# nncarlson/nka

Hardware: AMD Instinct MI355X
Metric: NKA updates/sec + achieved HBM GB/s at n=1e8, m=20 fp64; 1/2/4/8 GPUs (higher is better)
Workload: dtype f64

## Files before the change

### include/nka_hip_diag.h

```cpp
#ifndef NKA_HIP_DIAG_H
#define NKA_HIP_DIAG_H

#include "nka_hip_ext.h"
#include "nka_hip_vec.h"

#ifdef __cplusplus
extern "C" {
#endif

int nka_hip_set_tuning(nka_hip_t a, const char *key, int32_t value);

int nka_hip_set_grid(nka_hip_t a, int32_t pa_blocks_per_cu, int32_t pb_blocks_per_cu);

int nka_hip_debug_time_pa(nka_hip_t a, const double *f_dev, int32_t reps, float *ms_mean);

int nka_hip_debug_chain_sum(nka_hip_t a, const double *x_dev, const double *y_dev, int64_t n, double start, int32_t walk,
                            double *sum, float *ms);

int nka_hip_get_stamps(nka_hip_t a, double *out16);

int nka_hip_vec_set_tuning(nka_hip_vec_ws_t ws, const char *key, int32_t value);

#ifdef __cplusplus
}
#endif
// ... 2 lines not shown
```

### nka_amd/_lib.py

```python
from __future__ import annotations

import ctypes as C
import os
import subprocess

HERE = os.path.dirname(os.path.abspath(__file__))
_LIB = None

_i32p = C.POINTER(C.c_int32)
_dp = C.POINTER(C.c_double)
ALLREDUCE_FN = C.CFUNCTYPE(C.c_int, C.c_void_p, C.c_void_p, C.c_int32, C.c_void_p)
HOST_DOT_FN = C.CFUNCTYPE(C.c_double, C.c_void_p, C.c_int64, C.POINTER(C.c_double), C.POINTER(C.c_double))
HOST_ALLREDUCE_FN = C.CFUNCTYPE(C.c_int, C.c_void_p, C.POINTER(C.c_double), C.c_int32)

SIGNATURES = {
    "nka_hip_create": (C.c_int, [C.POINTER(C.c_void_p), C.c_int64, C.c_int32, C.c_double, C.c_int32, C.c_int32, C.c_void_p]),
    "nka_hip_destroy": (C.c_int, [C.c_void_p]),
    "nka_hip_clone": (C.c_int, [C.c_void_p, C.POINTER(C.c_void_p)]),
    "nka_hip_capture_safe": (C.c_int, [C.c_void_p]),
    "nka_hip_list_bound": (C.c_int, [C.c_void_p]),
    "nka_hip_set_stream": (C.c_int, [C.c_void_p, C.c_void_p]),
    "nka_hip_accel_update": (C.c_int, [C.c_void_p, C.c_void_p]),
    "nka_hip_accel_update_host": (C.c_int, [C.c_void_p, C.c_void_p]),
    "nka_hip_accel_update_swap": (C.c_int, [C.c_void_p, C.POINTER(C.c_void_p), C.POINTER(C.c_void_p)]),
# ... 109 lines not shown
    "nka_hip_batch_get_state": (C.c_int, [C.c_void_p, C.c_int32, _i32p, _i32p, _i32p, _i32p, _i32p, _i32p, _i32p, _dp, _dp]),
    "nka_hip_batch_get_reductions": (C.c_int, [C.c_void_p, C.c_int32, _dp]),
    "nka_hip_batch_get_w": (C.c_int, [C.c_void_p, C.c_int32, C.c_int32, _dp]),
    "nka_hip_batch_get_v": (C.c_int, [C.c_void_p, C.c_int32, C.c_int32, _dp]),
    "nka_hip_batch_state_digest": (C.c_int, [C.c_void_p, C.c_int32, C.POINTER(C.c_uint64)]),
}


DIAG_SIGNATURES = {
    "nka_hip_set_tuning": (C.c_int, [C.c_void_p, C.c_char_p, C.c_int32]),
    "nka_hip_set_grid": (C.c_int, [C.c_void_p, C.c_int32, C.c_int32]),
    "nka_hip_debug_time_pa": (C.c_int, [C.c_void_p, C.c_void_p, C.c_int32, C.POINTER(C.c_float)]),
    "nka_hip_debug_chain_sum": (C.c_int, [C.c_void_p, C.c_void_p, C.c_void_p, C.c_int64, C.c_double, C.c_int32,
                                          C.POINTER(C.c_double), C.POINTER(C.c_float)]),
    "nka_hip_get_stamps": (C.c_int, [C.c_void_p, _dp]),
    "nka_hip_vec_set_tuning": (C.c_int, [C.c_void_p, C.c_char_p, C.c_int32]),
}
_DIAG = None


def diag_lib_path() -> str:
    return os.environ.get("NKA_HIP_DIAG_LIB") or os.path.join(HERE, "libnka_hip_diag.so")


def load_diag() -> C.CDLL:
    global _DIAG
    if _DIAG is None:
        path = diag_lib_path()
        if not os.path.exists(path):
            raise RuntimeError(f"{path} not found: `make -C nka_amd/csrc diag` (or __graft_entry__.build())")
# ... 54 lines not shown
```

### nka_amd/csrc/handles.hpp

```cpp
#pragma once

#include "../../include/nka_hip.h"
#include "../../include/nka_hip_ext.h"
#include "../../include/nka_hip_vec.h"
#include "nka_ctl.hpp"
#include "host_logic.hpp"
#include "rccl_dl.hpp"

#include <hip/hip_runtime.h>

#include <cstdint>
#include <string>
#include <vector>

namespace nka_detail {
int set_error(int code, const std::string &msg);
std::string last_error();
bool &span_check_failed();
int check_device_span(const void *p, int64_t n, const char *what);
int check_device_span_i32(const void *p, int64_t n, const char *what);
void invalidate_span_cache();
void register_allocation(const void *p, size_t bytes, const void *owner);
void unregister_owner(const void *owner);
void unregister_allocation(const void *p);
// ... 51 lines not shown
  int num_cu = 256;
  int bpc[2] = {0, 0};
  char devname[64] = {0};
  int pa_pipe = -1;
  int pb_pipe = -1;
  int pb_flags = 0;
  int pb_tile = -1;
  int pb_tickets = -1;
  double *chain_pred = nullptr;
  void *chain_summ = nullptr;
  long long chain_cap = 0;
  int chain_many = -1;
  int chain_walk = 0;
  int fail_after_solve = 0;
  int prime_pad = -1;
  bool state_in_global = false;
  bool serial_solve = false;
  int sum_order = NKA_HIP_SUMS_AUTO;
  bool debug = false;
  nka_hip_allreduce_fn allreduce = nullptr;
  void *allreduce_ctx = nullptr;
  ncclComm_t comm = nullptr;
  nka::P2P p2p{};
  void *p2p_mail = nullptr;
  std::vector<void *> p2p_opened;
  void *p2p_dev = nullptr;
  int p2p_ranks = 0;
  bool p2p_fused = false;
  int pa_normed = 0;
  int shard_rank = -1, shard_n = 0;
// ... 32 lines not shown
```

### nka_amd/csrc/lab.hip

```cpp
#include "handles.hpp"
#include "nka_chain.hpp"
#include "../../include/nka_hip_diag.h"

#include <algorithm>
#include <string>

using namespace nka;
using namespace nka_detail;

extern "C" {

int nka_hip_get_stamps(nka_hip_t a, double *out16) {
  if (!a || !out16) return fail(NKA_HIP_EINVAL, "null argument");
  HIP_TRY(hipSetDevice(a->device));
  HIP_TRY(hipMemcpyAsync(out16, a->ctl.stamps(), sizeof(double) * kStamps, hipMemcpyDeviceToHost, a->stream));
  HIP_TRY(hipStreamSynchronize(a->stream));
  return 0;
}

int nka_hip_set_grid(nka_hip_t a, int32_t pa, int32_t pb) {
  if (!a) return fail(NKA_HIP_EINVAL, "null handle");
  const int32_t v[2] = {pa, pb};
  for (int i = 0; i < 2; i++) {
    if (v[i] < 0 || v[i] * a->num_cu > kMaxGrid) return fail(NKA_HIP_EINVAL, "blocks per CU out of range");
    a->bpc[i] = v[i];
  }
  return 0;
}

int nka_hip_debug_chain_sum(nka_hip_t a, const double *x, const double *y, int64_t n, double start, int32_t walk, double *sum,
// ... 69 lines not shown
    if (value != -1 && value != 0 && !(value > 200 && value <= 204))
      return fail(NKA_HIP_EINVAL, "pa_pipe: -1 (auto), 0 (every load of a tile in flight), 201..204 (rolling window, 1..4 blocks per CU)");
    a->pa_pipe = value;
  } else if (k == "pb_tile") {
    if (value != -1 && value != 1 && value != 2) return fail(NKA_HIP_EINVAL, "pb_tile: -1 (auto), 1, 2");
    a->pb_tile = value;
  } else if (k == "pb_tickets") {
    if (value != -1 && value != 0 && value != 1 && value != 2 && value != 4 && value != 8)
      return fail(NKA_HIP_EINVAL, "pb_tickets: -1 (auto), 0 (static tile mapping), 1, 2, 4, 8 (ticket counters)");
    a->pb_tickets = value;
  } else if (k == "fail_after_solve") {
    a->fail_after_solve = value != 0;
  } else if (k == "prime_pad") {
    if (value < -1 || value > 1) return fail(NKA_HIP_EINVAL, "prime_pad: -1, 0, 1");
    a->prime_pad = value;
  } else if (k == "chain_many") {
    if (value < -1 || value > 1) return fail(NKA_HIP_EINVAL, "chain_many: -1, 0, 1");
    a->chain_many = value;
  } else if (k == "chain_walk") {
    a->chain_walk = value != 0;
  } else if (k == "serial_solve") {
    a->serial_solve = value != 0;
  } else if (k == "list_word") {
    a->word_off = value == 0;
  } else {
    return fail(NKA_HIP_EINVAL, "unknown tuning key: " + k);
  }
  return 0;
}

// ... 13 lines not shown
```

### nka_amd/csrc/nka_ctl.hpp

```cpp
#pragma once

#include <cstddef>
#include <cstdint>

#if defined(__HIPCC__)
#include <hip/hip_runtime.h>
#define NKA_HOST_DEVICE __host__ __device__
#else
#define NKA_HOST_DEVICE
#endif

namespace nka {

enum {
  IC_SUBSPACE = 0,
  IC_PENDING = 1,
  IC_FIRST = 2,
  IC_LAST = 3,
  IC_FREE = 4,
  IC_NEW = 5,
  IC_NCOMB = 6,
  IC_PLAN_PENDING = 7,
  IC_PLAN_FIRST = 8,
  IC_PLAN_NOLDER = 9,
  IC_NRELAX = 10,
  IC_NORMED = 11,
  IC_HEADER = 16
};
enum { DC_VTOL = 0, DC_S = 1, DC_HEADER = 2 };
enum {
  PC_FIRST_W = 0,
  PC_NEW_W = 1,
  PC_NEW_V = 2,
  PC_OLD_W = 3,
  PC_OLD_V = 4,
  PC_WGT = 5,
  PC_HEADER = 8
};

constexpr int kMaxPerPass = 32;

// ... 54 lines not shown
```

### nka_amd/csrc/nka_device.hpp

```cpp
#pragma once

#include "nka_ctl.hpp"

#include <hip/hip_runtime.h>
#include <stdint.h>

#if defined(__HIP_DEVICE_COMPILE__) && !defined(__gfx950__)
#error "nka_device.hpp is written for gfx950 (CDNA4) only: v_permlane32_swap / v_permlane16_swap reductions, 160 KiB LDS, tile shapes measured on MI355X.  Build with --offload-arch=gfx950."
#endif

namespace nka {

constexpr int kBlock = 256;
constexpr int kWavesPerBlock = kBlock / 64;
constexpr int kMaxGrid = 4096;

#ifdef NKA_SOLVE_STAMPS
#define NKA_STAMP(ctl, i) do { if (threadIdx.x == 0) (ctl).stamps()[i] = (double)__builtin_amdgcn_s_memtime(); } while (0)
#define NKA_STAMP0(ctl, i) do { if (blockIdx.x == 0 && threadIdx.x == 0) (ctl).stamps()[i] = (double)__builtin_amdgcn_s_memtime(); } while (0)
#else
#define NKA_STAMP(ctl, i) do { } while (0)
#define NKA_STAMP0(ctl, i) do { } while (0)
#endif

// ... 144 lines not shown
  return __builtin_nontemporal_load(reinterpret_cast<const d2 *>(p));
}
__device__ __forceinline__ void st(double *p, double x) { __builtin_nontemporal_store(x, p); }
__device__ __forceinline__ void st(double *p, d2 x) { __builtin_nontemporal_store(x, reinterpret_cast<d2 *>(p)); }

__device__ __forceinline__ double ex(double x, int) { return x; }
__device__ __forceinline__ double ex(d2 x, int i) { return x[i]; }
__device__ __forceinline__ void setc(double &x, int, double val) { x = val; }
__device__ __forceinline__ void setc(d2 &x, int i, double val) { x[i] = val; }

__device__ __forceinline__ double pa_operand(double d, int normed, double s, double rs) {
  if (normed == 0) return d;
  if (s == 0.0) return 0.0;
  return (normed & 2) ? rs * d : d / s;
}

template <bool WGT, class V>
__device__ __forceinline__ double wgt_first(const V &om, int q, double a) {
  if constexpr (WGT) return ex(om, q) * a;
  else return a;
}
template <bool WGT>
__device__ __forceinline__ double wgt_at(const double *__restrict__ wgt, int64_t i, double a) {
  if constexpr (WGT) return wgt[i] * a;
  else return a;
}

constexpr int kOrdThreads = 256;
constexpr int kOrdChunkMax = 512;
constexpr int kOrdMaxMvec = 250;
// ... 269 lines not shown
```

### nka_amd/csrc/nka_hip.hip

```cpp
#include "handles.hpp"
#include "nka_kernels.hpp"

#include <dlfcn.h>

#include <algorithm>
#include <atomic>
#include <chrono>
#include <cmath>
#include <cstdio>
#include <cstdlib>
#include <cstring>
#include <map>
#include <mutex>
#include <set>
#include <string>
#include <vector>

using namespace nka;

namespace {
thread_local std::string g_err;
}

namespace nka_detail {
// ... 176 lines not shown
  else
    hipLaunchKernelGGL((k_dots<MAXL, VEC>), dim3(g), dim3(kBlock), 0, a->stream, a->ctl, a->vs, f, a->partials, pass, a->pa_normed);
  hipLaunchKernelGGL((k_finalize_dots<MAXL>), dim3(2 * MAXL + 2), dim3(kFinThreads), 0, a->stream, a->ctl,
                     a->partials, g, pass, npass * MAXL, pass * MAXL, a->p2p_fused ? a->p2p : P2P{}, a->pa_normed ? 1 : 0);
  return g;
}

template <int MAXL, int W>
int launch_dots_win_1(const nka_hip_state *a, const double *f, int bpc, int base, int pass, int ncover) {
  static const int occ = occupancy_of(k_dots_win<MAXL, W>);
  const int64_t ntile = a->n / (kBlock * 2);
  int64_t g = (int64_t)a->num_cu * std::min(occ, std::max(1, bpc));
  g = std::max<int64_t>(1, std::min<int64_t>(std::min<int64_t>(g, std::max<int64_t>(ntile, 1)), kMaxGrid));
  if (a->weighted)
    hipLaunchKernelGGL((k_dots_win<MAXL, W, true>), dim3((int)g), dim3(kBlock), 0, a->stream, a->ctl, a->vs, f, a->partials, base,
                       a->pa_normed);
  else
    hipLaunchKernelGGL((k_dots_win<MAXL, W>), dim3((int)g), dim3(kBlock), 0, a->stream, a->ctl, a->vs, f, a->partials, base, a->pa_normed);
  hipLaunchKernelGGL((k_finalize_dots<MAXL>), dim3(2 * MAXL + 2), dim3(kFinThreads), 0, a->stream, a->ctl,
                     a->partials, (int)g, pass, ncover < 0 ? MAXL : ncover, base, a->p2p_fused ? a->p2p : P2P{}, a->pa_normed ? 1 : 0);
  return (int)g;
}

template <int MAXL>
constexpr int win_ring() {
  return MAXL % 4 == 0 ? 4 : MAXL % 5 == 0 ? 5 : MAXL % 6 == 0 ? 6 : MAXL % 3 == 0 ? 3 : MAXL % 7 == 0 ? 7 : MAXL;
}

template <int MAXK>
constexpr int win_ring_pairs() {
  return MAXK % 2 == 0 ? 2 : MAXK % 3 == 0 ? 3 : MAXK % 5 == 0 ? 5 : MAXK % 7 == 0 ? 7 : MAXK;
}

#ifndef NKA_WINDOW_WIDTH_STEP
#define NKA_WINDOW_WIDTH_STEP 1
// ... 414 lines not shown
    e = hipGetLastError();
  }
  if (e != hipSuccess) {
    nka_hip_destroy(b);
    return fail(NKA_HIP_EHIP, std::string("nka_hip_clone: ") + hipGetErrorString(e));
  }
  b->pending = src->pending;
  b->list_ub = src->list_ub;
  b->bpc[0] = src->bpc[0];
  b->bpc[1] = src->bpc[1];
  b->pa_pipe = src->pa_pipe;
  b->pb_pipe = src->pb_pipe;
  b->pb_tile = src->pb_tile;
  b->pb_tickets = src->pb_tickets;
  b->prime_pad = src->prime_pad;
  b->chain_walk = src->chain_walk;
  b->chain_many = src->chain_many;
  b->chain_pred = nullptr; b->chain_summ = nullptr; b->chain_cap = 0;
  b->serial_solve = src->serial_solve;
  b->sum_order = src->sum_order;
  b->shard_rank = src->shard_rank;
  b->shard_n = src->shard_n;
  b->debug = src->debug;
  if (src->allreduce != rccl_allreduce && src->allreduce != p2p_allreduce) {
    b->allreduce = src->allreduce;
    b->allreduce_ctx = src->allreduce_ctx;
    b->needs_comm = src->needs_comm;
  } else {
    b->needs_comm = true;
  }
// ... 44 lines not shown
    if (a->relaxed_after.size() > 4096) a->relaxed_after.erase(a->relaxed_after.begin(), a->relaxed_after.begin() + 2048);
  }
  return 0;
}

int nka_hip_set_vec_tol(nka_hip_t a, double vtol) {
  if (!a) return fail(NKA_HIP_EINVAL, "null handle");
  if (!(vtol > 0.0)) return fail(NKA_HIP_EINVAL, "set_vec_tol: vtol must be > 0");
  HIP_TRY(hipSetDevice(a->device));
  a->vtol = vtol;
  HIP_TRY(hipMemcpyAsync(a->ctl.dc + DC_VTOL, &a->vtol, sizeof(double), hipMemcpyHostToDevice, a->stream));
  HIP_TRY(hipStreamSynchronize(a->stream));
  return 0;
}

static int enqueue_solve(nka_hip_t a, int mode, long long swap_w = kNoBuffer, long long swap_v = kNoBuffer, bool gather = false) {
  hipStream_t s = a->stream;
  const P2P x = gather ? a->p2p : P2P{};
  if (a->mvec + 1 <= kSolveWaveMax && !a->serial_solve) {
    const size_t sm = solve_wave_smem_bytes(a->mvec);
    const int nl = a->mvec + 1;
    const long long id_stride = (a->swapped || a->captured) ? 0 : (long long)a->vs.stride, id_vbase = buffer_offset(a, a->vs.v);
#define ROWS(NL) \
  hipLaunchKernelGGL((k_solve_rows<NL>), dim3(1), dim3(kSolveThreads), sm, s, a->ctl, mode, swap_w, swap_v, id_stride, id_vbase, x)
    if (nl <= 6) ROWS(6);
    else if (nl <= 11) ROWS(11);
    else if (nl <= 21) ROWS(21);
    else if (nl <= 33) ROWS(33);
    else if (nl <= 48) ROWS(48);
    else {
      if (!a->solve63_raised) {
        const hipError_t raised = hipFuncSetAttribute(reinterpret_cast<const void *>(k_solve_rows<63>),
                                                      hipFuncAttributeMaxDynamicSharedMemorySize,
                                                      (int)solve_wave_smem_bytes(kSolveWaveMax - 1));
        if (raised != hipSuccess) return fail(NKA_HIP_EHIP, std::string("raising the dynamic LDS limit failed: ") + hipGetErrorString(raised));
        a->solve63_raised = true;
      }
      ROWS(63);
    }
// ... 393 lines not shown
  a->p2p_fused = r.gather;
  enqueue_pa(a, f, vec, older_ub);
  a->p2p_fused = false;
  if (hipError_t e = hipGetLastError(); e != hipSuccess) {
    r.rc = fail(NKA_HIP_EHIP, std::string("accel_update: ") + hipGetErrorString(e));
    return r;
  }
  if (a->allreduce && !r.gather)
    if (int rc = a->allreduce(a->allreduce_ctx, a->ctl.red(), a->ctl.red_count(), a->stream)) r.rc = hook_failed(rc);
  return r;
}

static int update_impl(nka_hip_t a, double *f, long long swap_w, long long swap_v);
static int p2p_status_after_sync(nka_hip_t a);

int nka_hip_accel_update(nka_hip_t a, double *f) { return update_impl(a, f, kNoBuffer, kNoBuffer); }

static int update_impl(nka_hip_t a, double *f, long long swap_w, long long swap_v) {
  if (!a) return fail(NKA_HIP_EINVAL, "null handle");
  if (!f && a->n > 0) return fail(NKA_HIP_EINVAL, "accel_update: f is NULL");
  HIP_TRY(hipSetDevice(a->device));
  if (int rc = nka_detail::check_device_span(f, a->n, "accel_update: f")) return rc;
  if (swap_w == kNoBuffer && f && f == a->last_acc)
    return fail(NKA_HIP_EINVAL, "accel_update: that buffer is the accelerated f lent by the previous out-of-place update (read only: "
                                "it is the stored v of the pending pair); copy it, or go on with nka_hip_accel_update_swap");
  if (a->poisoned)
    return fail(NKA_HIP_ESTATE, "accel_update: an earlier update of this handle failed after its scalar step had been enqueued "
                                "(a HIP error): the lists on the device are ahead of the stored vectors.  Destroy the handle");
  if (a->swapped && f && held_by_library(a, f))
    return fail(NKA_HIP_EINVAL, "accel_update: that buffer is held by the library (a stored vector, or a buffer handed over to "
// ... 21 lines not shown
      if (hipStreamIsCapturing(s, &cs) != hipSuccess) (void)hipGetLastError();
      else if (cs != hipStreamCaptureStatusNone) {
        if (user_hook || a->host_dot)
          return fail(NKA_HIP_EINVAL, "accel_update: cannot be captured into a graph with a caller's all-reduce hook or dot product "
                                      "installed (host callbacks: a replay would not call them); the built-in RCCL hook and the "
                                      "peer-to-peer exchange can be captured");
        a->captured = a->word_off = true;
      }
    }
  }
  if (int rc = record(a, 0)) return rc;
  a->list_ub = list_bound_now(a);
  const int older_ub = a->pending ? std::max(a->list_ub - 1, 0) : a->list_ub;

  SumsResult sums{};
  switch (pick_sums_stage(a)) {
    case SumsStage::HostDot:        sums = sums_host_dot(a, f, mode); break;
    case SumsStage::ReferenceChain: sums = sums_reference_chain(a, f, mode, older_ub); break;
    case SumsStage::ReferenceOrder: sums = sums_reference_order(a, f, mode, older_ub); break;
    case SumsStage::Rounded:        sums = sums_rounded(a, f, vec, mode, older_ub); break;
    case SumsStage::Blocked:        sums = sums_blocked(a, f, vec, older_ub); break;
  }
  if (sums.rc) return sums.rc;
  mode |= sums.mode_bits;
  const bool solved = sums.solved, gather = sums.gather;
  if (int rc = record(a, 1)) return rc;

  RoctxRange range_tail("nka:solve + PB combine");
  if (!solved)
    if (int rc = enqueue_solve(a, mode, swap_w, swap_v, gather)) return rc;
  struct Poison {
    nka_hip_state *a;
    bool armed = true;
    ~Poison() { if (armed) a->poisoned = true; }
  } poison{a};
  if (a->fail_after_solve) {
    a->fail_after_solve = 0;
    return fail(NKA_HIP_EHIP, "accel_update: injected failure behind the scalar step (lab switch fail_after_solve)");
  }
  if (int rc = record(a, 2)) return rc;

  const int comb_ub = a->pending ? std::min(a->list_ub, (int)a->mvec) : a->list_ub;
  a->ctl.seq = (unsigned long long)(a->seq + 1);
  {
    Ctl &c = a->ctl;
    unsigned long long *const hw = c.hw;
    if (a->word_off) c.hw = nullptr;
    a->pb_flags = (swap_w != kNoBuffer ? (kPbNoStoreW | kPbNoStoreF) : 0);
    const int rc = enqueue_pb(a, f, vec, comb_ub);
    a->pb_flags = 0;
    c.hw = hw;
    if (rc) return rc;
  }
// ... 601 lines not shown
```

### nka_amd/csrc/nka_kernels.hpp

```cpp
#pragma once

#include "nka_chain.hpp"

namespace nka {


__global__ __launch_bounds__(128) void k_p2p_allreduce(P2P x, double *buf, int count) {
  const unsigned long long seq = *x.xseq;
  for (int i = threadIdx.x; i < count * x.n; i += blockDim.x) p2p_send_one(x, i % x.n, seq, i / x.n, buf[i / x.n]);
  __syncthreads();
  p2p_gather_block(x, buf, count);
}

template <int MAXL, int VEC, bool WGT = false>
__global__ __launch_bounds__(kBlock) void k_dots(Ctl ctl, Vecs vs, const double *__restrict__ f,
                                                 double *__restrict__ partials, int pass, int normed) {
  const double *wgt = WGT ? vs.w + ctl.pc[PC_WGT] : nullptr;
  using V = typename VecT<VEC>::type;
  constexpr int NACC = 2 * MAXL + 2;
  const int G = gridDim.x;
  const double s_n = normed ? sqrt(ctl.red()[0]) : 1.0, rs_n = 1.0 / s_n;
  const int pending = ctl.ic[IC_PLAN_PENDING];
  const int nolder = ctl.ic[IC_PLAN_NOLDER];
  const int base = pass * MAXL;
// ... 108 lines not shown
      acc = fma(wgt_at<WGT>(wgt, i, d), d, acc);
    }
  }
  const double one[1] = {acc};
  block_reduce_store<1>(one, partials, G);
}
__global__ __launch_bounds__(64) void k_norm_fin(Ctl ctl, const double *__restrict__ partials, int G) {
  double r = 0.0;
  for (int b = threadIdx.x; b < G; b += 64) r += partials[b];
  r = wave_sum(r);
  if (threadIdx.x == 0) ctl.red()[0] = ctl.ic[IC_PLAN_PENDING] ? r : 0.0;
}

template <int MAXL, int W, bool WGT = false>
__global__ __launch_bounds__(kBlock) void k_dots_win(Ctl ctl, Vecs vs, const double *__restrict__ f,
                                                     double *__restrict__ partials, int base, int normed) {
  constexpr int VEC = 2;
  using V = typename VecT<VEC>::type;
  constexpr int NACC = 2 * MAXL + 2;
  static_assert(MAXL % W == 0, "the ring must divide the stored vectors of a tile");
  NKA_STAMP0(ctl, 10);
  const int G = gridDim.x;
  const int pending = ctl.ic[IC_PLAN_PENDING];
  const double s_n = normed ? sqrt(ctl.red()[0]) : 1.0, rs_n = 1.0 / s_n;
  const int nolder = ctl.ic[IC_PLAN_NOLDER] - base;
  const long long *pw = ctl.plan_w() + base;
  const double *w1p = vs.w + ctl.pc[PC_FIRST_W];
  const double *w1 = pending ? w1p : f;
  const double *wgt = WGT ? vs.w + ctl.pc[PC_WGT] : nullptr;
  long long sl[MAXL];
#pragma unroll
  for (int j = 0; j < MAXL; j++) sl[j] = pw[j];
  const double *wk[MAXL];
#pragma unroll
  for (int j = 0; j < MAXL; j++) wk[j] = (j < nolder) ? vs.w + sl[j] : f;
  double acc[NACC];
#pragma unroll
  for (int a = 0; a < NACC; a++) acc[a] = 0.0;

  const int64_t ntile = vs.n / (kBlock * VEC);
#define DEAD_OFF(live, off) (off)
  V fv, w1v, omv = {}, ring[W];
  int64_t t = blockIdx.x;
  if (t < ntile) {
    const int64_t e = t * (kBlock * VEC) + threadIdx.x * VEC;
    fv = ld<VEC>(f + e);
    w1v = ld<VEC>(w1 + e);
    if constexpr (WGT) omv = ld<VEC>(wgt + e);
#pragma unroll
    for (int j = 0; j < W; j++) ring[j] = ld<VEC>(wk[j] + (DEAD_OFF(j < nolder, e)));
  }
  NKA_STAMP0(ctl, 11);
  for (; t < ntile; t += G) {
    const int64_t e = t * (kBlock * VEC) + threadIdx.x * VEC;
    const int64_t tn = (t + G < ntile) ? t + G : t;
    const int64_t en = tn * (kBlock * VEC) + threadIdx.x * VEC;
    double dq[VEC], fq[VEC];
#pragma unroll
    for (int q = 0; q < VEC; q++) {
      const double fx = ex(fv, q);
      const double dx = pa_operand(ex(w1v, q) - fx, normed, s_n, rs_n);
      dq[q] = wgt_first<WGT>(omv, q, dx);
      fq[q] = wgt_first<WGT>(omv, q, fx);
      acc[0] = fma(dq[q], dx, acc[0]);
      acc[1] = fma(fq[q], dx, acc[1]);
    }
    __builtin_amdgcn_sched_barrier(0);
    fv = ld<VEC>(f + en);
    w1v = ld<VEC>(w1 + en);
    if constexpr (WGT) omv = ld<VEC>(wgt + en);
#pragma unroll
    for (int j = 0; j < MAXL; j++) {
      const V x = ring[j % W];
      __builtin_amdgcn_sched_barrier(0);
      if (j + W < MAXL) ring[j % W] = ld<VEC>(wk[j + W] + (DEAD_OFF(j + W < nolder, e)));
      else ring[j % W] = ld<VEC>(wk[j + W - MAXL] + (DEAD_OFF(j + W - MAXL < nolder, en)));
      __builtin_amdgcn_sched_barrier(0);
#pragma unroll
      for (int q = 0; q < VEC; q++) {
        acc[2 + j] = fma(dq[q], ex(x, q), acc[2 + j]);
        acc[2 + MAXL + j] = fma(fq[q], ex(x, q), acc[2 + MAXL + j]);
      }
    }
  }
  if ((int)blockIdx.x == G - 1) {
    for (int64_t i = ntile * (kBlock * VEC) + threadIdx.x; i < vs.n; i += kBlock) {
      const double fx = f[i];
      const double d = pa_operand(w1[i] - fx, normed, s_n, rs_n);
      const double dw = wgt_at<WGT>(wgt, i, d), fw = wgt_at<WGT>(wgt, i, fx);
      acc[0] = fma(dw, d, acc[0]);
      acc[1] = fma(fw, d, acc[1]);
// ... 18 lines not shown
    const double x = w[i];
    if (!(x >= 0.0 && x <= __DBL_MAX__)) {
      bad++;
      if ((unsigned long long)i < first) first = (unsigned long long)i;
    }
  }
  if (bad) {
    atomicAdd(out, bad);
    atomicMin(out + 1, first);
  }
}

constexpr int kFinThreads = 64;
template <int MAXL>
__global__ __launch_bounds__(kFinThreads) void k_finalize_dots(Ctl ctl, const double *__restrict__ partials, int G,
                                                               int pass, int ncover, int base, P2P x, int keep0 = 0) {
  const int lane = threadIdx.x;
  const int c = blockIdx.x;
  const bool p2p = x.base != nullptr;
  const unsigned long long xs = p2p ? *x.xseq : 0ull;
  double r = 0.0;
  for (int b = lane; b < G; b += kFinThreads) r += partials[(size_t)c * G + b];
  r = wave_sum(r);
  const int nolder = ctl.ic[IC_PLAN_NOLDER];
  const int pending = ctl.ic[IC_PLAN_PENDING];
  if (pass == 0 && c == 0)
    for (int p = ncover + lane; p < ctl.mvec; p += kFinThreads) {
      if (p2p) {
        for (int q = 0; q < x.n; q++) {
          p2p_send_one(x, q, xs, 2 + p, 0.0);
          p2p_send_one(x, q, xs, 2 + ctl.mvec + p, 0.0);
        }
      } else {
        ctl.red()[2 + p] = 0.0;
        ctl.red()[2 + ctl.mvec + p] = 0.0;
      }
    }
  int dst = -1;
  bool live = false;
  if (c < 2) {
// ... 667 lines not shown

constexpr int kSolveWaveMax = 63;

__host__ __device__ inline size_t solve_wave_smem_bytes(int mvec) {
  const int nl = mvec + 1;
  size_t b = (lst_smem_bytes(mvec) + 15) / 16 * 16;
  b += (size_t)((nl + 1) * (nl + 1) + 3 * nl + (2 + 2 * mvec)) * sizeof(double);
  b += (size_t)(3 * nl + 1) * sizeof(int32_t);
  b = (b + 7) / 8 * 8;
  b += (size_t)(2 * (nl + 1)) * sizeof(long long);
  return b;
}

template <int NLMAX>
__global__ __launch_bounds__(kSolveThreads) void k_solve_rows(Ctl ctl, int mode, long long swap_w, long long swap_v,
                                                              long long id_stride, long long id_vbase, P2P x) {
  extern __shared__ __attribute__((aligned(16))) unsigned char smem[];
  const int lane = threadIdx.x;
  if (x.base != nullptr) p2p_gather_block(x, ctl.red(), ctl.red_count());
  const int m1 = ctl.m1(), NL = m1, LDA = NL + 1, M = ctl.mvec, nh = (m1 + 1) * (m1 + 1);
  Lst L;
  L.m1 = m1;
  L.mvec = M;
  L.h = reinterpret_cast<double *>(smem);
  L.c = L.h + nh;
  L.next = reinterpret_cast<int32_t *>(L.c + (m1 + 1));
  L.prev = L.next + (m1 + 1);
  double *A = reinterpret_cast<double *>(smem + (lst_smem_bytes(ctl.mvec) + 15) / 16 * 16);
  double *bb = A + (NL + 1) * LDA + 2 * NL;
  double *redL = bb + NL;
  int32_t *ord = reinterpret_cast<int32_t *>(redL + (2 + 2 * M));
  int32_t *psL = ord + 2 * NL;
  long long *wtL = reinterpret_cast<long long *>((reinterpret_cast<uintptr_t>(psL + NL + 1) + 7) / 8 * 8);
  long long *vtL = wtL + (m1 + 1);
  NKA_STAMP(ctl, 0);
  const int nolder = ctl.ic[IC_PLAN_NOLDER];
  {
    constexpr int kHB = 8;
    static_assert(kSolveWaveMax + 1 <= kSolveThreads, "lists: one load a lane");
    const double *gh = ctl.h(), *gred = ctl.red();
    double hreg[kHB], rreg[2], creg = 0.0;
    long long wtreg = 0, vtreg = 0;
    int32_t nreg = 0, preg = 0, psreg = 0;
#pragma unroll
    for (int k = 0; k < kHB; k++) hreg[k] = (lane + kSolveThreads * k < nh) ? gh[lane + kSolveThreads * k] : 0.0;
#pragma unroll
    for (int k = 0; k < 2; k++) rreg[k] = (lane + kSolveThreads * k < 2 + 2 * M) ? gred[lane + kSolveThreads * k] : 0.0;
    if (lane < m1 + 1) {
      creg = ctl.c()[lane];
      nreg = ctl.next()[lane];
      preg = ctl.prev()[lane];
// ... 13 lines not shown
    for (int k = 0; k < 2; k++)
      if (lane + kSolveThreads * k < 2 + 2 * M) redL[lane + kSolveThreads * k] = rreg[k];
    if (lane < m1 + 1) {
      L.c[lane] = creg;
      L.next[lane] = nreg;
      L.prev[lane] = preg;
      wtL[lane] = wtreg;
      vtL[lane] = vtreg;
    }
    if (lane < nolder) psL[lane] = psreg;
    for (int i = lane + kSolveThreads * kHB; i < nh; i += kSolveThreads) L.h[i] = gh[i];
  }
  lst_load_scalars(L, ctl);
  L.vtol = ctl.dc[DC_VTOL];
  const int entry_pending = L.pending;
  __syncthreads();
  NKA_STAMP(ctl, 1);
  const double vtol2 = L.vtol * L.vtol;

  const int entry_first = L.first;
  int normed = 0;
  double s = 0.0;
  if (L.pending) {
    s = sqrt(redL[0]);
    if (s == 0.0) lst_relax(L);
  }
  if (L.pending) normed = 1;
  {
    const double rs = 1.0 / s;
    for (int p = lane; p < nolder; p += kSolveThreads) {
      if (normed) L.H(L.first, psL[p]) = solve_nrm(redL[2 + p], s, rs, mode);
      L.c[psL[p]] = redL[2 + M + p];
    }
    if (normed && lane == 0) L.c[entry_first] = solve_nrm(redL[1], s, rs, mode);
  }
  __syncthreads();
  const int nl = normed ? 1 + nolder : 0;
  const int myord = normed ? (lane == 0 ? entry_first : (lane <= nolder ? psL[lane - 1] : 0)) : 0;
  NKA_STAMP(ctl, 2);
  const uint64_t listmask = (nl >= 64) ? ~0ull : ((1ull << nl) - 1);
  uint64_t alive = listmask;
  int capdrop = -1;
  bool forward_done = false;
  double ddr = 1.0;
  double Ldr = 1.0;
  double yr = 0.0;
  int nk = 0;

  if (normed) {
// ... 6 lines not shown
    }
    NKA_STAMP(ctl, 3);
    int kept = 0;
    bool open_ = true;
#pragma unroll
    for (int i = 0; i < NLMAX; i++) {
      bool keep = false;
      double Lii = 1.0;
      if (open_ && i < nl) {
        if (i == 0) {
          keep = true;
        } else if (kept + 1 > L.mvec) {
          capdrop = i;
          open_ = false;
        } else {
          const double hkk = readlane_f64(ddr, i);
          keep = hkk > vtol2;
          if (keep) Lii = sqrt(hkk);
        }
        if (!keep) alive &= ~(1ull << i);
      }
      if (keep) {
        kept++;
        if (lane == i) Ldr = Lii;
        const double l = a[i] / Lii;
        a[i] = l;
        if (lane > i && lane < nl) ddr = ddr - l * l;
#pragma unroll
        for (int q = i + 1; q < NLMAX; q++)
          a[q] = a[q] - l * readlane_f64(l, q);
      }
    }
    NKA_STAMP(ctl, 4);
    {
      double *const dump = A + NL * LDA + NL;
      const uint64_t rowbits = (lane < nl && ((alive >> lane) & 1)) ? (alive & ((1ull << lane) - 1)) : 0ull;
      if (lane <= nl) {
#pragma unroll
        for (int q = 0; q < NLMAX; q++) A[lane * LDA + (q < nl ? q : nl)] = a[q];
      }
#pragma unroll
      for (int q = 0; q < NLMAX; q++) {
        const int oq = __builtin_amdgcn_readlane(myord, q);
        double *const dst = ((rowbits >> q) & 1) ? &L.H(myord, oq) : dump;
        *dst = a[q];
      }
    }
    __syncthreads();
// ... 96 lines not shown
  __syncthreads();
  lst_prepend(L, slot);
  NKA_STAMP(ctl, 8);
  __syncthreads();
  lst_copy_out(L, ctl, kSolveThreads);
  if (lane == 0) {
    ctl.dc[DC_S] = s;
    if (entry_first != 0 && !normed && entry_pending) ctl.ic[IC_NRELAX] += 1;
    ctl.ic[IC_NEW] = slot;
    ctl.ic[IC_NCOMB] = nk;
    ctl.ic[IC_NORMED] = normed;
    lst_store_scalars(L, ctl);
    ctl.ic[IC_PLAN_PENDING] = L.pending;
    ctl.ic[IC_PLAN_FIRST] = L.first;
    ctl.ic[IC_PLAN_NOLDER] = nk;
  }
  NKA_STAMP(ctl, 9);
}

}
```

### nka_amd/nka.py

```python
from __future__ import annotations

import ctypes as C

import numpy as np

from . import _lib

FLAVOR_F08, FLAVOR_F08_VECTOR, FLAVOR_C = 0, 1, 2
FLAVOR_DEFAULT = -1
SUMS_AUTO, SUMS_REFERENCE_ORDER, SUMS_BLOCKED, SUMS_BLOCKED_ROUNDED = 0, 1, 2, 3


class NKAError(RuntimeError):
    pass


def _check(rc: int, what: str, L=None):
    if rc != 0:
        msg = (L or _lib.load()).nka_hip_last_error()
        raise NKAError(f"{what} failed ({rc}): {msg.decode() if msg else ''}")


class State:

# ... 350 lines not shown
        _check(self._L.nka_hip_get_timing(self._handle(), int(back), ms), "get_timing", self._L)
        return tuple(ms)

    def _need_diag(self, what):
        if not self._diag:
            raise NKAError(f"{what} exists only in the diagnostic build: construct the object with nka(diagnostic=True)")

    def set_grid(self, pa=0, pb=0):
        self._need_diag("set_grid")
        _check(self._L.nka_hip_set_grid(self._handle(), pa, pb), "set_grid", self._L)

    def set_tuning(self, key: str, value: int):
        self._need_diag("set_tuning")
        _check(self._L.nka_hip_set_tuning(self._handle(), key.encode(), int(value)), "set_tuning", self._L)

    def debug_chain_sum(self, x, y, start: float = 0.0, walk: bool = False, many: bool = False):
        self._need_diag("debug_chain_sum")
        assert x.dtype == y.dtype and x.numel() == y.numel() and x.is_contiguous() and y.is_contiguous()
        out, ms = C.c_double(), C.c_float()
        _check(self._L.nka_hip_debug_chain_sum(self._handle(), x.data_ptr(), y.data_ptr(), x.numel(), float(start),
                                               int(bool(walk)) | (2 if many else 0), C.byref(out), C.byref(ms)), "debug_chain_sum", self._L)
        return out.value, ms.value

    def device_info(self):
        name = C.create_string_buffer(64)
        ncu = C.c_int32()
        _check(self._L.nka_hip_device_info(self._handle(), name, C.byref(ncu)), "device_info", self._L)
        return name.value.decode(), ncu.value
```

Before: 134.9.

## Speculatively skip oldest stored vector in dots pass with device-side repair

When the history is full, the main dots kernel drops the oldest (about-to-be-evicted) vector from its streaming reads, pointing that slot at tile 0 so it hits cache instead of HBM. The solve detects whether that vector would have been needed (a zero norm, or it being the last kept column). If so, it flags a redo, and a repair dots pass plus a second solve run conditionally on the device. A hold counter disables skipping for mvec updates after a repair. This cuts one vector's worth of HBM traffic per update, at the cost of extra kernel launches that exit early when idle and occasional full repair passes.

```diff
diff --git a/include/nka_hip_diag.h b/include/nka_hip_diag.h
--- a/include/nka_hip_diag.h
+++ b/include/nka_hip_diag.h
@@ -9,6 +9,8 @@
 #endif
 
 int nka_hip_set_tuning(nka_hip_t a, const char *key, int32_t value);
+
+int nka_hip_get_skip_state(nka_hip_t a, int32_t out4[4]);
 
 int nka_hip_set_grid(nka_hip_t a, int32_t pa_blocks_per_cu, int32_t pb_blocks_per_cu);
 
diff --git a/nka_amd/_lib.py b/nka_amd/_lib.py
--- a/nka_amd/_lib.py
+++ b/nka_amd/_lib.py
@@ -147,6 +147,7 @@
     "nka_hip_debug_chain_sum": (C.c_int, [C.c_void_p, C.c_void_p, C.c_void_p, C.c_int64, C.c_double, C.c_int32,
                                           C.POINTER(C.c_double), C.POINTER(C.c_float)]),
     "nka_hip_get_stamps": (C.c_int, [C.c_void_p, _dp]),
+    "nka_hip_get_skip_state": (C.c_int, [C.c_void_p, C.POINTER(C.c_int32)]),
     "nka_hip_vec_set_tuning": (C.c_int, [C.c_void_p, C.c_char_p, C.c_int32]),
 }
 _DIAG = None
diff --git a/nka_amd/csrc/handles.hpp b/nka_amd/csrc/handles.hpp
--- a/nka_amd/csrc/handles.hpp
+++ b/nka_amd/csrc/handles.hpp
@@ -89,6 +89,8 @@
   int chain_walk = 0;
   int fail_after_solve = 0;
   int prime_pad = -1;
+  int skip_last = -1;
+  int pa_skip = 0;
   bool state_in_global = false;
   bool serial_solve = false;
   int sum_order = NKA_HIP_SUMS_AUTO;
diff --git a/nka_amd/csrc/lab.hip b/nka_amd/csrc/lab.hip
--- a/nka_amd/csrc/lab.hip
+++ b/nka_amd/csrc/lab.hip
@@ -14,6 +14,14 @@
   if (!a || !out16) return fail(NKA_HIP_EINVAL, "null argument");
   HIP_TRY(hipSetDevice(a->device));
   HIP_TRY(hipMemcpyAsync(out16, a->ctl.stamps(), sizeof(double) * kStamps, hipMemcpyDeviceToHost, a->stream));
+  HIP_TRY(hipStreamSynchronize(a->stream));
+  return 0;
+}
+
+int nka_hip_get_skip_state(nka_hip_t a, int32_t out4[4]) {
+  if (!a || !out4) return fail(NKA_HIP_EINVAL, "null argument");
+  HIP_TRY(hipSetDevice(a->device));
+  HIP_TRY(hipMemcpyAsync(out4, a->ctl.ic + IC_PLAN_SKIP, sizeof(int32_t) * 4, hipMemcpyDeviceToHost, a->stream));
   HIP_TRY(hipStreamSynchronize(a->stream));
   return 0;
 }
@@ -113,6 +121,9 @@
   } else if (k == "prime_pad") {
     if (value < -1 || value > 1) return fail(NKA_HIP_EINVAL, "prime_pad: -1, 0, 1");
     a->prime_pad = value;
+  } else if (k == "skip_last") {
+    if (value < -1 || value > 1) return fail(NKA_HIP_EINVAL, "skip_last: -1, 0, 1");
+    a->skip_last = value;
   } else if (k == "chain_many") {
     if (value < -1 || value > 1) return fail(NKA_HIP_EINVAL, "chain_many: -1, 0, 1");
     a->chain_many = value;
diff --git a/nka_amd/csrc/nka_ctl.hpp b/nka_amd/csrc/nka_ctl.hpp
--- a/nka_amd/csrc/nka_ctl.hpp
+++ b/nka_amd/csrc/nka_ctl.hpp
@@ -25,6 +25,10 @@
   IC_PLAN_NOLDER = 9,
   IC_NRELAX = 10,
   IC_NORMED = 11,
+  IC_PLAN_SKIP = 12,
+  IC_SKIP_HOLD = 13,
+  IC_REDO = 14,
+  IC_NREDO = 15,
   IC_HEADER = 16
 };
 enum { DC_VTOL = 0, DC_S = 1, DC_HEADER = 2 };
diff --git a/nka_amd/csrc/nka_device.hpp b/nka_amd/csrc/nka_device.hpp
--- a/nka_amd/csrc/nka_device.hpp
+++ b/nka_amd/csrc/nka_device.hpp
@@ -182,6 +182,12 @@
   if (s == 0.0) return 0.0;
   return (normed & 2) ? rs * d : d / s;
 }
+
+enum { kSkipMay = 1, kSkipRepair = 2 };
+__device__ __forceinline__ bool skip_last_planned(const Ctl &ctl, int skip, int pending, int nolder) {
+  return (skip & kSkipMay) && pending && nolder == ctl.mvec && ctl.ic[IC_PLAN_SKIP] != 0;
+}
+__device__ __forceinline__ bool skip_repair_idle(const Ctl &ctl, int skip) { return (skip & kSkipRepair) && ctl.ic[IC_REDO] == 0; }
 
 template <bool WGT, class V>
 __device__ __forceinline__ double wgt_first(const V &om, int q, double a) {
diff --git a/nka_amd/csrc/nka_hip.hip b/nka_amd/csrc/nka_hip.hip
--- a/nka_amd/csrc/nka_hip.hip
+++ b/nka_amd/csrc/nka_hip.hip
@@ -214,11 +214,13 @@
   g = std::max<int64_t>(1, std::min<int64_t>(std::min<int64_t>(g, std::max<int64_t>(ntile, 1)), kMaxGrid));
   if (a->weighted)
     hipLaunchKernelGGL((k_dots_win<MAXL, W, true>), dim3((int)g), dim3(kBlock), 0, a->stream, a->ctl, a->vs, f, a->partials, base,
-                       a->pa_normed);
+                       a->pa_normed, a->pa_skip);
   else
-    hipLaunchKernelGGL((k_dots_win<MAXL, W>), dim3((int)g), dim3(kBlock), 0, a->stream, a->ctl, a->vs, f, a->partials, base, a->pa_normed);
+    hipLaunchKernelGGL((k_dots_win<MAXL, W>), dim3((int)g), dim3(kBlock), 0, a->stream, a->ctl, a->vs, f, a->partials, base, a->pa_normed,
+                       a->pa_skip);
   hipLaunchKernelGGL((k_finalize_dots<MAXL>), dim3(2 * MAXL + 2), dim3(kFinThreads), 0, a->stream, a->ctl,
-                     a->partials, (int)g, pass, ncover < 0 ? MAXL : ncover, base, a->p2p_fused ? a->p2p : P2P{}, a->pa_normed ? 1 : 0);
+                     a->partials, (int)g, pass, ncover < 0 ? MAXL : ncover, base, a->p2p_fused ? a->p2p : P2P{}, a->pa_normed ? 1 : 0,
+                     a->pa_skip);
   return (int)g;
 }
 
@@ -663,6 +665,7 @@
   b->pb_tile = src->pb_tile;
   b->pb_tickets = src->pb_tickets;
   b->prime_pad = src->prime_pad;
+  b->skip_last = src->skip_last;
   b->chain_walk = src->chain_walk;
   b->chain_many = src->chain_many;
   b->chain_pred = nullptr; b->chain_summ = nullptr; b->chain_cap = 0;
@@ -737,7 +740,8 @@
   return 0;
 }
 
-static int enqueue_solve(nka_hip_t a, int mode, long long swap_w = kNoBuffer, long long swap_v = kNoBuffer, bool gather = false) {
+static int enqueue_solve(nka_hip_t a, int mode, long long swap_w = kNoBuffer, long long swap_v = kNoBuffer, bool gather = false,
+                         int skip = 0) {
   hipStream_t s = a->stream;
   const P2P x = gather ? a->p2p : P2P{};
   if (a->mvec + 1 <= kSolveWaveMax && !a->serial_solve) {
@@ -745,7 +749,8 @@
     const int nl = a->mvec + 1;
     const long long id_stride = (a->swapped || a->captured) ? 0 : (long long)a->vs.stride, id_vbase = buffer_offset(a, a->vs.v);
 #define ROWS(NL) \
-  hipLaunchKernelGGL((k_solve_rows<NL>), dim3(1), dim3(kSolveThreads), sm, s, a->ctl, mode, swap_w, swap_v, id_stride, id_vbase, x)
+  hipLaunchKernelGGL((k_solve_rows<NL>), dim3(1), dim3(kSolveThreads), sm, s, a->ctl, mode, swap_w, swap_v, id_stride, id_vbase, x, \
+                     skip)
     if (nl <= 6) ROWS(6);
     else if (nl <= 11) ROWS(11);
     else if (nl <= 21) ROWS(21);
@@ -1169,6 +1174,16 @@
 static int update_impl(nka_hip_t a, double *f, long long swap_w, long long swap_v);
 static int p2p_status_after_sync(nka_hip_t a);
 
+constexpr double kSkipLastMinBytes = 4.8e7;
+static bool skip_last_applies(const nka_hip_state *a, SumsStage stage, int vec, int older_ub) {
+  if (a->skip_last == 0) return false;
+  if (stage != SumsStage::Rounded && stage != SumsStage::Blocked) return false;
+  if (a->allreduce || a->host_dot || a->serial_solve) return false;
+  if (a->mvec < 2 || a->mvec > kMaxPerPass || vec != 2 || older_ub != a->mvec) return false;
+  if (a->pa_pipe != -1 && a->pa_pipe != 201) return false;
+  return a->skip_last > 0 || 8.0 * (double)a->n >= kSkipLastMinBytes;
+}
+
 int nka_hip_accel_update(nka_hip_t a, double *f) { return update_impl(a, f, kNoBuffer, kNoBuffer); }
 
 static int update_impl(nka_hip_t a, double *f, long long swap_w, long long swap_v) {
@@ -1220,13 +1235,17 @@
   const int older_ub = a->pending ? std::max(a->list_ub - 1, 0) : a->list_ub;
 
   SumsResult sums{};
-  switch (pick_sums_stage(a)) {
+  const SumsStage stage = pick_sums_stage(a);
+  const bool skip = skip_last_applies(a, stage, vec, older_ub);
+  a->pa_skip = skip ? kSkipMay : 0;
+  switch (stage) {
     case SumsStage::HostDot:        sums = sums_host_dot(a, f, mode); break;
     case SumsStage::ReferenceChain: sums = sums_reference_chain(a, f, mode, older_ub); break;
     case SumsStage::ReferenceOrder: sums = sums_reference_order(a, f, mode, older_ub); break;
     case SumsStage::Rounded:        sums = sums_rounded(a, f, vec, mode, older_ub); break;
     case SumsStage::Blocked:        sums = sums_blocked(a, f, vec, older_ub); break;
   }
+  a->pa_skip = 0;
   if (sums.rc) return sums.rc;
   mode |= sums.mode_bits;
   const bool solved = sums.solved, gather = sums.gather;
@@ -1234,7 +1253,7 @@
 
   RoctxRange range_tail("nka:solve + PB combine");
   if (!solved)
-    if (int rc = enqueue_solve(a, mode, swap_w, swap_v, gather)) return rc;
+    if (int rc = enqueue_solve(a, mode, swap_w, swap_v, gather, skip ? kSkipMay : 0)) return rc;
   struct Poison {
     nka_hip_state *a;
     bool armed = true;
@@ -1243,6 +1262,14 @@
   if (a->fail_after_solve) {
     a->fail_after_solve = 0;
     return fail(NKA_HIP_EHIP, "accel_update: injected failure behind the scalar step (lab switch fail_after_solve)");
+  }
+  if (skip) {
+    a->pa_skip = kSkipRepair;
+    a->pa_normed = stage == SumsStage::Rounded ? ((mode & kSolveRcp) ? 3 : 1) : 0;
+    launch_dots_win(1, a, f, 1, a->mvec - 1, 1, a->mvec);
+    a->pa_skip = a->pa_normed = 0;
+    HIP_TRY(hipGetLastError());
+    if (int rc = enqueue_solve(a, mode, swap_w, swap_v, false, kSkipRepair)) return rc;
   }
   if (int rc = record(a, 2)) return rc;
 
diff --git a/nka_amd/csrc/nka_kernels.hpp b/nka_amd/csrc/nka_kernels.hpp
--- a/nka_amd/csrc/nka_kernels.hpp
+++ b/nka_amd/csrc/nka_kernels.hpp
@@ -146,16 +146,20 @@
 
 template <int MAXL, int W, bool WGT = false>
 __global__ __launch_bounds__(kBlock) void k_dots_win(Ctl ctl, Vecs vs, const double *__restrict__ f,
-                                                     double *__restrict__ partials, int base, int normed) {
+                                                     double *__restrict__ partials, int base, int normed, int skip) {
   constexpr int VEC = 2;
   using V = typename VecT<VEC>::type;
   constexpr int NACC = 2 * MAXL + 2;
   static_assert(MAXL % W == 0, "the ring must divide the stored vectors of a tile");
+  if (skip_repair_idle(ctl, skip)) return;
   NKA_STAMP0(ctl, 10);
   const int G = gridDim.x;
   const int pending = ctl.ic[IC_PLAN_PENDING];
   const double s_n = normed ? sqrt(ctl.red()[0]) : 1.0, rs_n = 1.0 / s_n;
-  const int nolder = ctl.ic[IC_PLAN_NOLDER] - base;
+  const int nplan = ctl.ic[IC_PLAN_NOLDER];
+  const bool skip_last = skip_last_planned(ctl, skip, pending, nplan);
+  const int nolder = nplan - (skip_last ? 1 : 0) - base;
+  const bool last_far = skip_last && ctl.mvec - base == MAXL;
   const long long *pw = ctl.plan_w() + base;
   const double *w1p = vs.w + ctl.pc[PC_FIRST_W];
   const double *w1 = pending ? w1p : f;
@@ -171,22 +175,25 @@
   for (int a = 0; a < NACC; a++) acc[a] = 0.0;
 
   const int64_t ntile = vs.n / (kBlock * VEC);
-#define DEAD_OFF(live, off) (off)
+#define DEAD_OFF(j, off, off_far) ((j) == MAXL - 1 ? (off_far) : (off))
   V fv, w1v, omv = {}, ring[W];
   int64_t t = blockIdx.x;
   if (t < ntile) {
     const int64_t e = t * (kBlock * VEC) + threadIdx.x * VEC;
+    const int64_t ef = (last_far ? 0 : t) * (kBlock * VEC) + threadIdx.x * VEC;
     fv = ld<VEC>(f + e);
     w1v = ld<VEC>(w1 + e);
     if constexpr (WGT) omv = ld<VEC>(wgt + e);
 #pragma unroll
-    for (int j = 0; j < W; j++) ring[j] = ld<VEC>(wk[j] + (DEAD_OFF(j < nolder, e)));
+    for (int j = 0; j < W; j++) ring[j] = ld<VEC>(wk[j] + (DEAD_OFF(j, e, ef)));
   }
   NKA_STAMP0(ctl, 11);
   for (; t < ntile; t += G) {
     const int64_t e = t * (kBlock * VEC) + threadIdx.x * VEC;
     const int64_t tn = (t + G < ntile) ? t + G : t;
     const int64_t en = tn * (kBlock * VEC) + threadIdx.x * VEC;
+    const int64_t ef = (last_far ? 0 : t) * (kBlock * VEC) + threadIdx.x * VEC;
+    const int64_t enf = (last_far ? 0 : tn) * (kBlock * VEC) + threadIdx.x * VEC;
     double dq[VEC], fq[VEC];
 #pragma unroll
     for (int q = 0; q < VEC; q++) {
@@ -205,8 +212,8 @@
     for (int j = 0; j < MAXL; j++) {
       const V x = ring[j % W];
       __builtin_amdgcn_sched_barrier(0);
-      if (j + W < MAXL) ring[j % W] = ld<VEC>(wk[j + W] + (DEAD_OFF(j + W < nolder, e)));
-      else ring[j % W] = ld<VEC>(wk[j + W - MAXL] + (DEAD_OFF(j + W - MAXL < nolder, en)));
+      if (j + W < MAXL) ring[j % W] = ld<VEC>(wk[j + W] + (DEAD_OFF(j + W, e, ef)));
+      else ring[j % W] = ld<VEC>(wk[j + W - MAXL] + (DEAD_OFF(j + W - MAXL, en, enf)));
       __builtin_amdgcn_sched_barrier(0);
 #pragma unroll
       for (int q = 0; q < VEC; q++) {
@@ -255,7 +262,9 @@
 constexpr int kFinThreads = 64;
 template <int MAXL>
 __global__ __launch_bounds__(kFinThreads) void k_finalize_dots(Ctl ctl, const double *__restrict__ partials, int G,
-                                                               int pass, int ncover, int base, P2P x, int keep0 = 0) {
+                                                               int pass, int ncover, int base, P2P x, int keep0 = 0,
+                                                               int skip = 0) {
+  if (skip_repair_idle(ctl, skip)) return;
   const int lane = threadIdx.x;
   const int c = blockIdx.x;
   const bool p2p = x.base != nullptr;
@@ -263,8 +272,9 @@
   double r = 0.0;
   for (int b = lane; b < G; b += kFinThreads) r += partials[(size_t)c * G + b];
   r = wave_sum(r);
-  const int nolder = ctl.ic[IC_PLAN_NOLDER];
   const int pending = ctl.ic[IC_PLAN_PENDING];
+  const int nplan = ctl.ic[IC_PLAN_NOLDER];
+  const int nolder = nplan - (skip_last_planned(ctl, skip, pending, nplan) ? 1 : 0);
   if (pass == 0 && c == 0)
     for (int p = ncover + lane; p < ctl.mvec; p += kFinThreads) {
       if (p2p) {
@@ -962,9 +972,10 @@
 
 template <int NLMAX>
 __global__ __launch_bounds__(kSolveThreads) void k_solve_rows(Ctl ctl, int mode, long long swap_w, long long swap_v,
-                                                              long long id_stride, long long id_vbase, P2P x) {
+                                                              long long id_stride, long long id_vbase, P2P x, int skip) {
   extern __shared__ __attribute__((aligned(16))) unsigned char smem[];
   const int lane = threadIdx.x;
+  if (skip_repair_idle(ctl, skip)) return;
   if (x.base != nullptr) p2p_gather_block(x, ctl.red(), ctl.red_count());
   const int m1 = ctl.m1(), NL = m1, LDA = NL + 1, M = ctl.mvec, nh = (m1 + 1) * (m1 + 1);
   Lst L;
@@ -983,6 +994,7 @@
   long long *vtL = wtL + (m1 + 1);
   NKA_STAMP(ctl, 0);
   const int nolder = ctl.ic[IC_PLAN_NOLDER];
+  const int hold_in = ctl.ic[IC_SKIP_HOLD];
   {
     constexpr int kHB = 8;
     static_assert(kSolveWaveMax + 1 <= kSolveThreads, "lists: one load a lane");
@@ -1026,6 +1038,8 @@
   lst_load_scalars(L, ctl);
   L.vtol = ctl.dc[DC_VTOL];
   const int entry_pending = L.pending;
+  const bool skipped = !(skip & kSkipRepair) && skip_last_planned(ctl, skip, entry_pending, nolder);
+  bool redo = false;
   __syncthreads();
   NKA_STAMP(ctl, 1);
   const double vtol2 = L.vtol * L.vtol;
@@ -1037,6 +1051,7 @@
     s = sqrt(redL[0]);
     if (s == 0.0) lst_relax(L);
   }
+  if (skipped && s == 0.0) redo = true;
   if (L.pending) normed = 1;
   {
     const double rs = 1.0 / s;
@@ -1045,6 +1060,13 @@
       L.c[psL[p]] = redL[2 + M + p];
     }
     if (normed && lane == 0) L.c[entry_first] = solve_nrm(redL[1], s, rs, mode);
+  }
+  if (redo) {
+    if (lane == 0) {
+      ctl.ic[IC_REDO] = 1;
+      ctl.ic[IC_NREDO] += 1;
+    }
+    return;
   }
   __syncthreads();
   const int nl = normed ? 1 + nolder : 0;
@@ -1081,6 +1103,7 @@
           capdrop = i;
           open_ = false;
         } else {
+          if (skipped && i == nl - 1) redo = true;
           const double hkk = readlane_f64(ddr, i);
           keep = hkk > vtol2;
           if (keep) Lii = sqrt(hkk);
@@ -1099,6 +1122,13 @@
       }
     }
     NKA_STAMP(ctl, 4);
+    if (redo) {
+      if (lane == 0) {
+        ctl.ic[IC_REDO] = 1;
+        ctl.ic[IC_NREDO] += 1;
+      }
+      return;
+    }
     {
       double *const dump = A + NL * LDA + NL;
       const uint64_t rowbits = (lane < nl && ((alive >> lane) & 1)) ? (alive & ((1ull << lane) - 1)) : 0ull;
@@ -1225,6 +1255,13 @@
     ctl.ic[IC_PLAN_PENDING] = L.pending;
     ctl.ic[IC_PLAN_FIRST] = L.first;
     ctl.ic[IC_PLAN_NOLDER] = nk;
+    int hold = hold_in > 0 ? hold_in - 1 : 0;
+    if (skip & kSkipRepair) {
+      hold = M;
+      ctl.ic[IC_REDO] = 0;
+    }
+    ctl.ic[IC_SKIP_HOLD] = hold;
+    ctl.ic[IC_PLAN_SKIP] = hold == 0 ? 1 : 0;
   }
   NKA_STAMP(ctl, 9);
 }
diff --git a/nka_amd/nka.py b/nka_amd/nka.py
--- a/nka_amd/nka.py
+++ b/nka_amd/nka.py
@@ -388,6 +388,12 @@
         self._need_diag("set_tuning")
         _check(self._L.nka_hip_set_tuning(self._handle(), key.encode(), int(value)), "set_tuning", self._L)
 
+    def skip_state(self):
+        self._need_diag("skip_state")
+        out = (C.c_int32 * 4)()
+        _check(self._L.nka_hip_get_skip_state(self._handle(), out), "get_skip_state", self._L)
+        return tuple(out)
+
     def debug_chain_sum(self, x, y, start: float = 0.0, walk: bool = False, many: bool = False):
         self._need_diag("debug_chain_sum")
         assert x.dtype == y.dtype and x.numel() == y.numel() and x.is_contiguous() and y.is_contiguous()
```

New measurement: 136.6 (median of 6 runs). 1.2% higher.
